# Gorilla-Lab-SCUT/GeoA3

Measured on AMD Instinct MI355X. Metric: attack-iterations/sec (B=250, N=1024), higher is better.
Workload: dtype f32; 1 GPU; configs[1]: PointNet 1024-pt, 250 instances sharded over 1 GPU(s) (250 on rank 0), full GeoA3 (CE + CD 1.0 + HD 0.1 + curvature 1.0 k=16), untargeted; instances_per_gpu=250, global_batch=250, npoint=1024, knn=16, classes=40, wide_mode=f16x2, presteps=150, parallelism=instance-sharded x1

## Files before the change

geoa3_amd/build.py:

```python
from __future__ import annotations

import concurrent.futures
import hashlib
import os
import shutil
import subprocess
import sys

HERE = os.path.dirname(os.path.abspath(__file__))
CSRC = os.path.join(HERE, "csrc")
LIBDIR = os.path.join(HERE, "lib")
OBJDIR = os.path.join(LIBDIR, "obj")
LIB = os.path.join(LIBDIR, "libgeoa3_hip.so")
ARCH = "gfx950"
FLAGS = ["-O3", "-std=c++17", "-fPIC", "--offload-arch=" + ARCH, "-fno-gpu-rdc", "-Wall", "-Wno-unused-function"]


def _hipcc() -> str:
    for c in (os.environ.get("HIPCC"), shutil.which("hipcc"), "/opt/rocm/bin/hipcc"):
        if c and os.path.exists(c):
            return c
    raise RuntimeError("hipcc not found: the HIP library cannot be built")


_NOSLP = ["-fno-slp-vectorize", "-fno-vectorize"]
SLP_FILES = ("pointnet_gemm.hip",)
FILE_FLAGS = {f: list(_NOSLP) for f in sorted(os.listdir(CSRC)) if f.endswith(".hip") and f not in SLP_FILES}
for _f in ("pointnet2_sa.hip", "pointnet2_sa2.hip", "pointnet2_sa2b.hip", "geom_filter.hip", "geom_grid.hip"):
    FILE_FLAGS[_f] = ["-fno-honor-nans"] + _NOSLP


def sources():
    return sorted(os.path.join(CSRC, f) for f in os.listdir(CSRC) if f.endswith(".hip"))


_HIPCC_VERSION = None


def hipcc_version() -> str:
    global _HIPCC_VERSION
    if _HIPCC_VERSION is None:
        r = subprocess.run([_hipcc(), "--version"], capture_output=True, text=True)
        _HIPCC_VERSION = (r.stdout + r.stderr).strip()
    return _HIPCC_VERSION


def _digest(path: str, flags=None) -> str:
    h = hashlib.sha1()
    for p in [path] + sorted(os.path.join(CSRC, f) for f in os.listdir(CSRC) if f.endswith(".h")) + [
            os.path.join(HERE, "..", "include", "geoa3_hip.h"), os.path.join(HERE, "..", "include", "geoa3_hip_debug.h")]:
        with open(p, "rb") as f:
            h.update(f.read())
    h.update(" ".join(flags or FLAGS).encode())
    h.update(hipcc_version().encode())
    h.update(repr((ISA_GUARD_ALL, sorted(ISA_GUARDS.items()))).encode())
    return h.hexdigest()


def _compile(src: str, force: bool, objdir: str = OBJDIR, flags=None) -> str:
    flags_in = tuple(flags or ())
    flags = list(flags or FLAGS)
    if "--no-file-flags" in flags:
        flags.remove("--no-file-flags")
    elif os.path.basename(src) in os.environ.get("GEOA3_NO_FILE_FLAGS_FOR", "").split(",") and objdir != OBJDIR:
        pass
    else:
        flags += FILE_FLAGS.get(os.path.basename(src), [])
    extra = os.environ.get("GEOA3_EXTRA_FILE_FLAGS", "")
    if extra and objdir != OBJDIR:
        names, _, fl = extra.partition(":")
        if os.path.basename(src) in names.split(",") and fl not in flags:
            flags.append(fl)
    obj = os.path.join(objdir, os.path.basename(src) + ".o")
    stamp = obj + ".sha1"
    dig = _digest(src, flags)
    if not force and os.path.exists(obj) and os.path.exists(stamp) and open(stamp).read() == dig:
        return obj
    guarded = ("--no-file-flags" not in (flags_in or ()) and
               not (objdir != OBJDIR and os.environ.get("GEOA3_NO_FILE_FLAGS_FOR")))
    import tempfile
    with tempfile.TemporaryDirectory(dir=objdir) as d:
        tmp_obj = os.path.join(d, os.path.basename(src) + ".o")
        cmd = [_hipcc()] + flags + (["-save-temps=obj"] if guarded else []) + ["-c", src, "-o", tmp_obj]
        r = subprocess.run(cmd, capture_output=True, text=True, cwd=d)
        if r.returncode != 0:
            raise RuntimeError("hipcc failed for %s:\n%s\n%s" % (src, r.stdout, r.stderr))
        if r.stderr.strip():
            sys.stderr.write(r.stderr)
        if guarded:
            base = os.path.splitext(os.path.basename(src))[0]
            asm_file = os.path.join(d, "%s-hip-amdgcn-amd-amdhsa-%s.s" % (base, ARCH))
            if not os.path.exists(asm_file):
                raise RuntimeError("ISA guard: hipcc -save-temps left no device assembly for %s (looked for %s)" % (src, asm_file))
            _isa_guard_asm(src, open(asm_file).read(), flags)
        os.replace(tmp_obj, obj)
    with open(stamp, "w") as f:
        f.write(dig)
    return obj


ISA_GUARDS = {"pointnet_conv_chain.hip": ("conv_bwd_chain_kernel", r"v_pk_(mul|fma|add)_f32"),
              "pointnet2_ops.hip": ("fps_kernel", r"v_pk_(mul|fma|add)_f32"),
              "geom_loss.hip": ("geo_fused_kernel", r"v_pk_(mul|fma|add)_f32")}


ISA_GUARD_ALL = r"(?i)v_pk_(mul|fma|add)_f32\w*[^\n]*\bop_sel\s*[:=]\s*\[[^\]]*1"


GUARD_SELFTEST_SOURCE = r"""
// MUST be refused by the ISA guard: packed FP32 arithmetic whose LOW result reads the HIGH half of a source register pair
#include <hip/hip_runtime.h>
typedef float f2 __attribute__((ext_vector_type(2)));
__global__ void guard_selftest_kernel(const f2* a, const f2* b, f2* out) {
  const int i = blockIdx.x * blockDim.x + threadIdx.x;
  const f2 x = a[i], y = b[i];
  const f2 ys = {y.y, y.x};          // swapped halves: v_pk_fma_f32 ... op_sel:[0,1,0] op_sel_hi:[1,0,1]
  out[i] = x * ys + x;
}
"""


def isa_guard_selftest() -> str:
    import tempfile
    with tempfile.TemporaryDirectory() as d:
        src = os.path.join(d, "guard_selftest.hip")
        with open(src, "w") as f:
            f.write(GUARD_SELFTEST_SOURCE)
        try:
            _isa_guard(src, FLAGS)
        except RuntimeError as e:
            if "ISA guard" in str(e) and "op_sel" in str(e):
                return str(e)
            raise
    raise AssertionError("the ISA guard accepted a source that holds packed FP32 arithmetic with op_sel on a source operand: "
                         "either this hipcc (%s) no longer forms v_pk_*_f32 ... op_sel from the self-test source, or it prints "
                         "it in a way ISA_GUARD_ALL misses -- look at the disassembly before trusting the build"
                         % hipcc_version().splitlines()[0])


def _isa_guard(src: str, flags) -> None:
    import tempfile
    with tempfile.TemporaryDirectory() as d:
        out = os.path.join(d, "guard.s")
        cmd = [_hipcc()] + [f for f in flags if f != "-fPIC"] + ["-S", "--cuda-device-only", "-o", out, src]
        r = subprocess.run(cmd, capture_output=True, text=True)
        if r.returncode != 0:
            raise RuntimeError("ISA guard: hipcc -S failed for %s:\n%s" % (src, r.stderr))
        asm = open(out).read()
    _isa_guard_asm(src, asm, flags)


def _isa_guard_asm(src: str, asm: str, flags) -> None:
    import re
    kernel, pattern = ISA_GUARDS.get(os.path.basename(src), (None, None))
    hit = re.search(ISA_GUARD_ALL, asm)
    if hit:
        raise RuntimeError("ISA guard: %s holds '%s' (NOTEBOOK 5a: packed FP32 with op_sel reads a zero operand in lanes 48-63 "
                           "beside matrix-core wavefronts); keep the two values apart (an opaque asm barrier) or compile the "
                           "file with %s" % (os.path.basename(src), hit.group(0).strip(), " ".join(_NOSLP)))
    if kernel is None:
        return
    found = list(re.finditer(r"^(_Z\w*%s\w*):" % kernel, asm, re.M))
    if not found:
        raise RuntimeError("ISA guard: kernel %s not found in %s" % (kernel, src))
    for m in found:
        body = asm[m.end():]
        body = body[:body.index("s_endpgm")]
        hit = re.search(pattern, body)
        if hit:
            raise RuntimeError("ISA guard: %s holds %s (NOTEBOOK 5a: wrong values beside other wavefronts on its SIMDs); compile "
                               "%s with %s" % (m.group(1), hit.group(0), os.path.basename(src),
                                               FILE_FLAGS.get(os.path.basename(src))))


def build(force: bool = False, verbose: bool = True, extra_flags=(), libdir: str = LIBDIR) -> str:
    objdir, lib = os.path.join(libdir, "obj"), os.path.join(libdir, "libgeoa3_hip.so")
    flags = FLAGS + list(extra_flags)
    os.makedirs(objdir, exist_ok=True)
    srcs = sources()
    with concurrent.futures.ThreadPoolExecutor(max_workers=min(6, len(srcs))) as ex:
        objs = list(ex.map(lambda s: _compile(s, force, objdir, flags), srcs))
    newest = max(os.path.getmtime(o) for o in objs)
    if force or not os.path.exists(lib) or os.path.getmtime(lib) < newest:
        cmd = [_hipcc(), "-shared", "-fPIC", "--offload-arch=" + ARCH, "-o", lib] + objs
        r = subprocess.run(cmd, capture_output=True, text=True)
        if r.returncode != 0:
            raise RuntimeError("link failed:\n%s\n%s" % (r.stdout, r.stderr))
    if verbose:
        print("built", lib, "%.0f KB" % (os.path.getsize(lib) / 1024))
    return lib


if __name__ == "__main__":
    if "--variant" in sys.argv:
        i = sys.argv.index("--variant")
        build(force="--force" in sys.argv, libdir=os.path.abspath(sys.argv[i + 1]),
              extra_flags=[f for f in sys.argv[i + 2:] if f.startswith("-") and f != "--force"])
    else:
        build(force="--force" in sys.argv)
```

geoa3_amd/csrc/pointnet_conv_chain.hip:

```cpp
#include "pointnet_kernels.h"

namespace {

__device__ __forceinline__ void cc_writelane(int& d, int v, int l) {
  asm("v_writelane_b32 %0, %1, %2" : "+v"(d) : "s"(v), "n"(l));
}

constexpr int CC_PITCH = 64 * 2 + 16;
constexpr int CC_BLK = 2 * 64 * CC_PITCH;

__device__ __forceinline__ void cc_mm(const float (&xin)[64], const unsigned char* arow, bool live, f32x16 (&acc)[2][2],
                                      unsigned& Ex) {
#pragma unroll
  for (int c = 0; c < 2; ++c)
#pragma unroll
    for (int t = 0; t < 2; ++t)
#pragma unroll
      for (int r = 0; r < 16; ++r) acc[c][t][r] = 0.f;
  Ex = 14u;
#pragma unroll
  for (int c = 0; c < 4; ++c) {
    const float* x = xin + 16 * c;
    float m = 0.f;
#pragma unroll
    for (int u = 0; u < 16; ++u) m = fmaxf(m, __builtin_fabsf(x[u]));
    const unsigned E = sf_exp(wave_max(live ? m : 0.f));
    if (E > Ex) {
      if (c > 0) {
        const unsigned d = E - Ex;
        const float f = d > 126u ? 0.f : __uint_as_float((127u - d) << 23);
#pragma unroll
        for (int cb = 0; cb < 2; ++cb)
#pragma unroll
          for (int t = 0; t < 2; ++t)
#pragma unroll
            for (int r = 0; r < 16; ++r) acc[cb][t][r] *= f;
      }
      Ex = E;
    }
    const float sx = sf_scale(Ex);
    half8 xh[2], xl[2];
#pragma unroll
    for (int j = 0; j < 8; ++j) {
      float v0 = x[j] * sx, v1 = x[8 + j] * sx;
      geoa3_swap32(v0, v1);
      const _Float16 h0 = (_Float16)v0, h1 = (_Float16)v1;
      xh[0][j] = h0;
      xl[0][j] = (_Float16)(v0 - (float)h0);
      xh[1][j] = h1;
      xl[1][j] = (_Float16)(v1 - (float)h1);
    }
#pragma unroll
    for (int t = 0; t < 2; ++t) {
      const half8 wh = *reinterpret_cast<const half8*>(arow + t * 32 * CC_PITCH + c * 32);
      const half8 wl = *reinterpret_cast<const half8*>(arow + t * 32 * CC_PITCH + c * 32 + 64 * CC_PITCH);
#pragma unroll
      for (int cb = 0; cb < 2; ++cb) {
        acc[cb][t] = __builtin_amdgcn_mfma_f32_32x32x16_f16(wh, xh[cb], acc[cb][t], 0, 0, 0);
        acc[cb][t] = __builtin_amdgcn_mfma_f32_32x32x16_f16(wh, xl[cb], acc[cb][t], 0, 0, 0);
        acc[cb][t] = __builtin_amdgcn_mfma_f32_32x32x16_f16(wl, xh[cb], acc[cb][t], 0, 0, 0);
      }
    }
  }
}

__device__ __forceinline__ void cc_rows(const f32x16 (&acc)[2][2], float (&out)[64]) {
#pragma unroll
  for (int t = 0; t < 2; ++t)
#pragma unroll
    for (int g = 0; g < 4; ++g)
#pragma unroll
      for (int i = 0; i < 4; ++i) {
        float v0 = acc[0][t][4 * g + i], v1 = acc[1][t][4 * g + i];
        geoa3_swap32(v0, v1);
        out[t * 32 + 8 * g + i] = v0;
        out[t * 32 + 8 * g + 4 + i] = v1;
      }
}

__device__ __forceinline__ void cc_wload(const float* W, bool kcontig, int tid, float (&wv)[16], float* s_red) {
  float m = 0.f;
#pragma unroll
  for (int i = 0; i < 16; ++i) {
    wv[i] = W[tid + 256 * i];
    m = fmaxf(m, __builtin_fabsf(wv[i]));
  }
  (void)kcontig;
  m = wave_max(m);
  if ((tid & 63) == 0) s_red[tid >> 6] = m;
}
__device__ __forceinline__ unsigned cc_wsplit(const float (&wv)[16], bool kcontig, int tid, const float* s_red,
                                              unsigned char* s_wh) {
  const unsigned Ew = sf_exp(fmaxf(fmaxf(s_red[0], s_red[1]), fmaxf(s_red[2], s_red[3])));
  const float sw = sf_scale(Ew);
#pragma unroll
  for (int i = 0; i < 16; ++i) {
    const int e = tid + 256 * i;
    const int co = kcontig ? e >> 6 : e & 63, k = kcontig ? e & 63 : e >> 6;
    const float v = wv[i] * sw;
    const _Float16 h = (_Float16)v;
    *reinterpret_cast<_Float16*>(s_wh + co * CC_PITCH + k * 2) = h;
    *reinterpret_cast<_Float16*>(s_wh + 64 * CC_PITCH + co * CC_PITCH + k * 2) = (_Float16)(v - (float)h);
  }
  return Ew;
}

template <int NS, bool FIRST, int COL>
__global__ __launch_bounds__(256) __attribute__((amdgpu_waves_per_eu(2, 2))) void conv_chain_kernel(ConvChainArgs a) {
  extern __shared__ __attribute__((aligned(16))) unsigned char cc_smem[];
  constexpr int NBLK = NS - 1 + COL / 64;
  float4* s_w1 = reinterpret_cast<float4*>(cc_smem + NBLK * CC_BLK);
  float* s_red = reinterpret_cast<float*>(s_w1 + 64);
  const int tid = threadIdx.x, lane = tid & 63, wave = tid >> 6;
  const int b = blockIdx.y;
  const int nblk256 = (a.N + 255) >> 8;
  if (FIRST && tid < 64) s_w1[tid] = make_float4(a.w1[3 * tid], a.w1[3 * tid + 1], a.w1[3 * tid + 2], a.b1[tid]);

  float biasv[NBLK];
  unsigned Ew[NBLK];
  {
    float wv[NBLK][16];
#pragma unroll
    for (int blk = 0; blk < NBLK; ++blk) {
      const int s = blk < NS - 1 ? blk : NS - 1, rb = blk - s;
      const float* W = a.st[s].W + (size_t)b * a.st[s].sWb + (size_t)rb * 4096;
      biasv[blk] = a.st[s].bias[rb * 64 + lane];
      cc_wload(W, true, tid, wv[blk], s_red + blk * 4);
    }
    __syncthreads();
#pragma unroll
    for (int blk = 0; blk < NBLK; ++blk) {
      Ew[blk] = cc_wsplit(wv[blk], true, tid, s_red + blk * 4, cc_smem + blk * CC_BLK);
    }
    __syncthreads();
  }
  for (int cblk = blockIdx.x; cblk < nblk256; cblk += gridDim.x) {
  const int col = cblk * 256 + wave * 64 + lane;
  const bool live = col < a.N, wave_live = cblk * 256 + wave * 64 < a.N;
  const unsigned long long livemask = __builtin_amdgcn_ballot_w64(live);
  const size_t mword = ((size_t)b * ((a.N + 63) >> 6) + (size_t)(cblk * 4 + wave));
  float o[64];
  if (FIRST) {
    const float* xp = a.x3 + (size_t)b * 3 * a.N + (live ? col : a.N - 1);
    const float x0 = xp[0], x1 = xp[a.N], x2 = xp[2 * (size_t)a.N];
    float p0 = x0, p1 = x1, p2 = x2;
    if (a.T3) {
      const float* t = a.T3 + (size_t)b * 9;
      p0 = x0 * t[0] + x1 * t[3] + x2 * t[6];
      p1 = x0 * t[1] + x1 * t[4] + x2 * t[7];
      p2 = x0 * t[2] + x1 * t[5] + x2 * t[8];
    }
#pragma unroll
    for (int u = 0; u < 64; ++u) o[u] = fmaxf(pn_first_layer(s_w1[u], p0, p1, p2), 0.f);
  } else {
    const float* X = a.X + (size_t)b * a.sXb;
    const unsigned xc = (unsigned)(live ? col : a.N - 1);
#pragma unroll
    for (int u = 0; u < 64; ++u) o[u] = (X + (size_t)u * a.ldX)[xc];
  }

#pragma unroll
  for (int blk = 0; blk < NBLK; ++blk) {
    const int s = blk < NS - 1 ? blk : NS - 1, rb = blk - s;
    const bool last = s == NS - 1;
    const ChainStage& st = a.st[s];
    const unsigned char* arow = cc_smem + blk * CC_BLK + (lane & 31) * CC_PITCH + (lane >> 5) * 16;

    f32x16 acc[2][2];
    unsigned Ex;
    cc_mm(o, arow, live, acc, Ex);
    const float unscale = sf_unscale(Ex) * sf_unscale(Ew[blk]);

    float res[64];
    int mlo = 0, mhi = 0;
    cc_rows(acc, res);
#pragma unroll
    for (int row = 0; row < 64; ++row) {
      float r = res[row] * unscale;
      r += __int_as_float(__builtin_amdgcn_readlane(__float_as_int(biasv[blk]), row));
      r = fmaxf(r, 0.f);
      const unsigned long long mk = __builtin_amdgcn_ballot_w64(r > 0.f) & livemask;
      cc_writelane(mlo, (int)(unsigned)mk, row);
      cc_writelane(mhi, (int)(unsigned)(mk >> 32), row);
      res[row] = r;
    }
    if (wave_live)
      st.Ymask[mword * st.Co + rb * 64 + lane] = ((unsigned long long)(unsigned)mhi << 32) | (unsigned)mlo;
    if (st.Y && live) {
      float* Y = st.Y + (size_t)b * st.sYb + (size_t)rb * 64 * a.N;
#pragma unroll
      for (int r = 0; r < 64; ++r) (Y + (size_t)r * a.N)[(unsigned)col] = res[r];
    }
    if (!last) {
#pragma unroll
      for (int r = 0; r < 64; ++r) o[r] = res[r];
    }
  }
  }
}

__global__ __launch_bounds__(256) __attribute__((amdgpu_waves_per_eu(2, 2))) void conv_bwd_chain_kernel(ConvBwdChainArgs a) {
  extern __shared__ __attribute__((aligned(16))) unsigned char cc_smem[];
  float4* s_w1 = reinterpret_cast<float4*>(cc_smem + 3 * CC_BLK);
  float* s_red = reinterpret_cast<float*>(s_w1 + 64);
  float* s_part = s_red + 12;
  const int tid = threadIdx.x, lane = tid & 63, wave = tid >> 6;
  const int cblk = blockIdx.x, b = blockIdx.y;
  const int col = cblk * 256 + wave * 64 + lane;
  const bool live = col < a.N, wave_live = cblk * 256 + wave * 64 < a.N;
  const unsigned xc = (unsigned)(live ? col : a.N - 1);
  const size_t mword = ((size_t)b * ((a.N + 63) >> 6) + (size_t)(cblk * 4 + wave)) * 64;

  float o[64], xb[64];
  {
    const float* X = a.Xa + (size_t)b * 64 * a.N;
#pragma unroll
    for (int u = 0; u < 64; ++u) o[u] = (X + (size_t)u * a.N)[xc];
  }
  const float* xp = a.x3 + (size_t)b * 3 * a.N + xc;
  const float x0 = xp[0], x1 = xp[a.N], x2 = xp[2 * (size_t)a.N];
  float p0 = x0, p1 = x1, p2 = x2;
  if (a.T3) {
    const float* t = a.T3 + (size_t)b * 9;
    p0 = x0 * t[0] + x1 * t[3] + x2 * t[6];
    p1 = x0 * t[1] + x1 * t[4] + x2 * t[7];
    p2 = x0 * t[2] + x1 * t[5] + x2 * t[8];
  }
  if (tid < 64) s_w1[tid] = make_float4(a.w1[3 * tid], a.w1[3 * tid + 1], a.w1[3 * tid + 2], a.b1[tid]);
  const unsigned long long zmv = wave_live ? a.Zmask[mword + lane] : 0ull;

  unsigned Ew[3];
  {
    float wv[3][16];
    cc_wload(a.Wa + (size_t)b * a.sWa, false, tid, wv[0], s_red);
    cc_wload(a.Wb, false, tid, wv[1], s_red + 4);
    cc_wload(a.W2t, true, tid, wv[2], s_red + 8);
    __syncthreads();
    Ew[0] = cc_wsplit(wv[0], false, tid, s_red, cc_smem);
    Ew[1] = cc_wsplit(wv[1], false, tid, s_red + 4, cc_smem + CC_BLK);
    Ew[2] = cc_wsplit(wv[2], true, tid, s_red + 8, cc_smem + 2 * CC_BLK);
    __syncthreads();
  }
  {
    const float* X = a.Xb + (size_t)b * 64 * a.N;
#pragma unroll
    for (int u = 0; u < 64; ++u) xb[u] = (X + (size_t)u * a.N)[xc];
  }
  const unsigned char* arow = cc_smem + (lane & 31) * CC_PITCH + (lane >> 5) * 16;
  f32x16 acc[2][2];
  unsigned Ex;
  float res[64];
  cc_mm(o, arow, live, acc, Ex);
  {
    const float un = sf_unscale(Ex) * sf_unscale(Ew[0]);
    cc_rows(acc, o);
#pragma unroll
    for (int r = 0; r < 64; ++r) o[r] *= un;
  }
  cc_mm(xb, arow + CC_BLK, live, acc, Ex);
  {
    const float un = sf_unscale(Ex) * sf_unscale(Ew[1]);
    cc_rows(acc, res);
    const unsigned sh = lane & 31;
#pragma unroll
    for (int r = 0; r < 64; ++r) {
      float v = res[r] * un;
      v += o[r];
      const unsigned mlo = (unsigned)__builtin_amdgcn_readlane((int)(unsigned)zmv, r);
      const unsigned mhi = (unsigned)__builtin_amdgcn_readlane((int)(unsigned)(zmv >> 32), r);
      o[r] = (((lane < 32 ? mlo : mhi) >> sh) & 1u) ? v : 0.f;
    }
  }
  cc_mm(o, arow + 2 * CC_BLK, live, acc, Ex);
  float q0 = 0.f, q1 = 0.f, q2 = 0.f;
  {
    const float un = sf_unscale(Ex) * sf_unscale(Ew[2]);
    cc_rows(acc, res);
    if (live) {
#pragma unroll
      for (int r = 0; r < 64; ++r) {
        float v = res[r] * un;
        const float4 w = s_w1[r];
        v = pn_first_layer(w, p0, p1, p2) > 0.f ? v : 0.f;
        q0 = fmaf(w.x, v, q0);
        q1 = fmaf(w.y, v, q1);
        q2 = fmaf(w.z, v, q2);
      }
    }
  }
  float d0 = q0, d1 = q1, d2 = q2;
  if (a.T3) {
    const float* t = a.T3 + (size_t)b * 9;
    d0 = fmaf(t[2], q2, fmaf(t[1], q1, t[0] * q0));
    d1 = fmaf(t[5], q2, fmaf(t[4], q1, t[3] * q0));
    d2 = fmaf(t[8], q2, fmaf(t[7], q1, t[6] * q0));
  }
  if (live) {
    float* dxp = a.dx + (size_t)b * 3 * a.N + col;
    dxp[0] = d0;
    dxp[a.N] = d1;
    dxp[2 * (size_t)a.N] = d2;
  }
  if (a.dTpart) {
    const float prod[9] = {x0 * q0, x0 * q1, x0 * q2, x1 * q0, x1 * q1, x1 * q2, x2 * q0, x2 * q1, x2 * q2};
#pragma unroll
    for (int i = 0; i < 9; ++i) {
      const float v = wave_sum(prod[i]);
      if (lane == 0) s_part[wave * 9 + i] = v;
    }
    __syncthreads();
    if (tid < 9) {
      a.dTpart[((size_t)b * gridDim.x + cblk) * GEOA3_DT_PITCH + tid] = s_part[tid] + s_part[9 + tid] + s_part[18 + tid] + s_part[27 + tid];
    }
  }
}

template <int NS, bool FIRST, int COL>
void launch_chain(const ConvChainArgs& a, hipStream_t s) {
  constexpr int NBLK = NS - 1 + COL / 64;
  const size_t lds = (size_t)NBLK * CC_BLK + 64 * 16 + NBLK * 4 * sizeof(float);
  auto kern = conv_chain_kernel<NS, FIRST, COL>;
  (void)hipFuncSetAttribute(reinterpret_cast<const void*>(kern), hipFuncAttributeMaxDynamicSharedMemorySize, (int)lds);
  const int nblk = (a.N + 255) / 256;
  const int gx = (size_t)nblk * a.B > 768 ? (nblk + 1) / 2 : nblk;
  hipLaunchKernelGGL(kern, dim3(gx, a.B), dim3(256), lds, s, a);
}

}

int launch_conv_chain(const ConvChainArgs& a, hipStream_t s) {
  if (a.ns < 1 || a.ns > 3 || a.B <= 0 || a.N <= 0) return GEOA3_EINVAL;
  for (int i = 0; i < a.ns; ++i) {
    if (!a.st[i].W || !a.st[i].bias || !a.st[i].Ymask) return GEOA3_EINVAL;
    if (a.st[i].Co != (i + 1 < a.ns ? 64 : 128)) return GEOA3_ENOSUPPORT;
  }
  const bool first = a.x3 != nullptr;
  if (first ? (!a.w1 || !a.b1) : !a.X) return GEOA3_EINVAL;
  if (a.ns == 3 && first) launch_chain<3, true, 128>(a, s);
  else if (a.ns == 1 && first) launch_chain<1, true, 128>(a, s);
  else if (a.ns == 2 && !first) launch_chain<2, false, 128>(a, s);
  else return GEOA3_ENOSUPPORT;
  GEOA3_CHECK_LAUNCH();
  return GEOA3_OK;
}

int launch_conv_bwd_chain(const ConvBwdChainArgs& a, hipStream_t s) {
  if (!a.Xa || !a.Wa || !a.Xb || !a.Wb || !a.Zmask || !a.W2t || !a.x3 || !a.w1 || !a.b1 || !a.dx || a.B <= 0 || a.N <= 0)
    return GEOA3_EINVAL;
  const size_t lds = (size_t)3 * CC_BLK + 64 * 16 + (12 + 36) * sizeof(float);
  (void)hipFuncSetAttribute(reinterpret_cast<const void*>(conv_bwd_chain_kernel), hipFuncAttributeMaxDynamicSharedMemorySize,
                            (int)lds);
  hipLaunchKernelGGL(conv_bwd_chain_kernel, dim3((a.N + 255) / 256, a.B), dim3(256), lds, s, a);
  GEOA3_CHECK_LAUNCH();
  return GEOA3_OK;
}
```

Baseline: 622.8 iterations/s of a 250-instance batch.

## Use 512-thread workgroups looping over column blocks in PointNet conv chain kernels

For large batches, the forward and backward conv-chain kernels now launch 8-wave workgroups that loop over several column blocks. Each workgroup fetches, scales and splits the per-instance weights into LDS once and reuses them across more columns, which cuts repeated weight loading and setup. The backward kernel now holds the weight preamble once and accumulates dT partials across iterations. The forward epilogue can fuse the Y store into the mask loop when all lanes are live. It also adds compile-time CC_CUT switches for profiling, plus build-guard updates to check both kernel instances. The trade-off is fewer, larger workgroups, which means more register and LDS pressure per group and possibly less occupancy or overlap.

```diff
diff --git a/geoa3_amd/build.py b/geoa3_amd/build.py
--- a/geoa3_amd/build.py
+++ b/geoa3_amd/build.py
@@ -53,7 +53,7 @@
             h.update(f.read())
     h.update(" ".join(flags or FLAGS).encode())
     h.update(hipcc_version().encode())
-    h.update(repr((ISA_GUARD_ALL, sorted(ISA_GUARDS.items()))).encode())
+    h.update(repr((ISA_GUARD_ALL, sorted(ISA_GUARDS.items()), sorted(ISA_GUARD_INSTANCES.items()))).encode())
     return h.hexdigest()
 
 
@@ -69,8 +69,8 @@
     extra = os.environ.get("GEOA3_EXTRA_FILE_FLAGS", "")
     if extra and objdir != OBJDIR:
         names, _, fl = extra.partition(":")
-        if os.path.basename(src) in names.split(",") and fl not in flags:
-            flags.append(fl)
+        if os.path.basename(src) in names.split(","):
+            flags += [f for f in fl.split() if f not in flags]
     obj = os.path.join(objdir, os.path.basename(src) + ".o")
     stamp = obj + ".sha1"
     dig = _digest(src, flags)
@@ -99,9 +99,10 @@
     return obj
 
 
-ISA_GUARDS = {"pointnet_conv_chain.hip": ("conv_bwd_chain_kernel", r"v_pk_(mul|fma|add)_f32"),
+ISA_GUARDS = {"pointnet_conv_chain.hip": (r"conv_bwd_chain(_wg8)?_kernel", r"v_pk_(mul|fma|add)_f32"),
               "pointnet2_ops.hip": ("fps_kernel", r"v_pk_(mul|fma|add)_f32"),
               "geom_loss.hip": ("geo_fused_kernel", r"v_pk_(mul|fma|add)_f32")}
+ISA_GUARD_INSTANCES = {"pointnet_conv_chain.hip": 2}
 
 
 ISA_GUARD_ALL = r"(?i)v_pk_(mul|fma|add)_f32\w*[^\n]*\bop_sel\s*[:=]\s*\[[^\]]*1"
@@ -161,8 +162,9 @@
     if kernel is None:
         return
     found = list(re.finditer(r"^(_Z\w*%s\w*):" % kernel, asm, re.M))
-    if not found:
-        raise RuntimeError("ISA guard: kernel %s not found in %s" % (kernel, src))
+    if len(found) < ISA_GUARD_INSTANCES.get(os.path.basename(src), 1):
+        raise RuntimeError("ISA guard: kernel %s: %d instance(s) found in %s, %d expected" % (
+            kernel, len(found), src, ISA_GUARD_INSTANCES.get(os.path.basename(src), 1)))
     for m in found:
         body = asm[m.end():]
         body = body[:body.index("s_endpgm")]
diff --git a/geoa3_amd/csrc/pointnet_conv_chain.hip b/geoa3_amd/csrc/pointnet_conv_chain.hip
--- a/geoa3_amd/csrc/pointnet_conv_chain.hip
+++ b/geoa3_amd/csrc/pointnet_conv_chain.hip
@@ -1,6 +1,14 @@
 #include "pointnet_kernels.h"
 
+#ifndef GEOA3_CC_CUT
+#define GEOA3_CC_CUT 0
+#endif
+
 namespace {
+
+constexpr int CC_CUT = GEOA3_CC_CUT;
+
+__device__ __forceinline__ void cc_keep(float v) { asm volatile("" ::"v"(v)); }
 
 __device__ __forceinline__ void cc_writelane(int& d, int v, int l) {
   asm("v_writelane_b32 %0, %1, %2" : "+v"(d) : "s"(v), "n"(l));
@@ -78,24 +86,29 @@
       }
 }
 
-__device__ __forceinline__ void cc_wload(const float* W, bool kcontig, int tid, float (&wv)[16], float* s_red) {
+template <int NT>
+__device__ __forceinline__ void cc_wfetch(const float* W, int tid, float (&wv)[4096 / NT]) {
+#pragma unroll
+  for (int i = 0; i < 4096 / NT; ++i) wv[i] = W[tid + NT * i];
+}
+template <int NT>
+__device__ __forceinline__ void cc_wmax(const float (&wv)[4096 / NT], int tid, float* s_red) {
   float m = 0.f;
 #pragma unroll
-  for (int i = 0; i < 16; ++i) {
-    wv[i] = W[tid + 256 * i];
-    m = fmaxf(m, __builtin_fabsf(wv[i]));
-  }
-  (void)kcontig;
+  for (int i = 0; i < 4096 / NT; ++i) m = fmaxf(m, __builtin_fabsf(wv[i]));
   m = wave_max(m);
   if ((tid & 63) == 0) s_red[tid >> 6] = m;
 }
-__device__ __forceinline__ unsigned cc_wsplit(const float (&wv)[16], bool kcontig, int tid, const float* s_red,
+template <int NT>
+__device__ __forceinline__ unsigned cc_wsplit(const float (&wv)[4096 / NT], bool kcontig, int tid, const float* s_red,
                                               unsigned char* s_wh) {
-  const unsigned Ew = sf_exp(fmaxf(fmaxf(s_red[0], s_red[1]), fmaxf(s_red[2], s_red[3])));
+  float wm = fmaxf(fmaxf(s_red[0], s_red[1]), fmaxf(s_red[2], s_red[3]));
+  if (NT == 512) wm = fmaxf(wm, fmaxf(fmaxf(s_red[4], s_red[5]), fmaxf(s_red[6], s_red[7])));
+  const unsigned Ew = sf_exp(wm);
   const float sw = sf_scale(Ew);
 #pragma unroll
-  for (int i = 0; i < 16; ++i) {
-    const int e = tid + 256 * i;
+  for (int i = 0; i < 4096 / NT; ++i) {
+    const int e = tid + NT * i;
     const int co = kcontig ? e >> 6 : e & 63, k = kcontig ? e & 63 : e >> 6;
     const float v = wv[i] * sw;
     const _Float16 h = (_Float16)v;
@@ -105,44 +118,76 @@
   return Ew;
 }
 
-template <int NS, bool FIRST, int COL>
-__global__ __launch_bounds__(256) __attribute__((amdgpu_waves_per_eu(2, 2))) void conv_chain_kernel(ConvChainArgs a) {
+__device__ __forceinline__ void cc_xload(const float* X, size_t ld, unsigned xc, float (&o)[64]) {
+#pragma unroll
+  for (int u = 0; u < 64; ++u) {
+    if (CC_CUT & 2) o[u] = __uint_as_float(0x3c000000u + ((xc & 63u) << 8) + 8192u * (unsigned)u);
+    else o[u] = (X + (size_t)u * ld)[xc];
+  }
+}
+
+template <bool STORE>
+__device__ __forceinline__ void cc_epilogue(float (&res)[64], float unscale, float biasv, unsigned long long livemask, int& mlo,
+                                            int& mhi, float* Y, size_t ldY, unsigned col) {
+#pragma unroll
+  for (int row = 0; row < 64; ++row) {
+    float r = res[row] * unscale;
+    r += __int_as_float(__builtin_amdgcn_readlane(__float_as_int(biasv), row));
+    r = fmaxf(r, 0.f);
+    const unsigned long long mk = __builtin_amdgcn_ballot_w64(r > 0.f) & livemask;
+    cc_writelane(mlo, (int)(unsigned)mk, row);
+    cc_writelane(mhi, (int)(unsigned)(mk >> 32), row);
+    res[row] = r;
+    if (STORE) (Y + (size_t)row * ldY)[col] = r;
+  }
+}
+
+template <int NS, bool FIRST, int COL, int WPG>
+__global__ __launch_bounds__(64 * WPG) __attribute__((amdgpu_waves_per_eu(2, 2))) void conv_chain_kernel(ConvChainArgs a) {
   extern __shared__ __attribute__((aligned(16))) unsigned char cc_smem[];
+  constexpr int NT = 64 * WPG;
   constexpr int NBLK = NS - 1 + COL / 64;
   float4* s_w1 = reinterpret_cast<float4*>(cc_smem + NBLK * CC_BLK);
   float* s_red = reinterpret_cast<float*>(s_w1 + 64);
   const int tid = threadIdx.x, lane = tid & 63, wave = tid >> 6;
   const int b = blockIdx.y;
-  const int nblk256 = (a.N + 255) >> 8;
+  const int nblkw = (a.N + NT - 1) / NT;
+  const bool never = a.N < 0;
   if (FIRST && tid < 64) s_w1[tid] = make_float4(a.w1[3 * tid], a.w1[3 * tid + 1], a.w1[3 * tid + 2], a.b1[tid]);
 
+  float o[64];
   float biasv[NBLK];
   unsigned Ew[NBLK];
-  {
-    float wv[NBLK][16];
+  float wv[NBLK][4096 / NT];
+#pragma unroll
+  for (int blk = 0; blk < NBLK; ++blk) {
+    const int s = blk < NS - 1 ? blk : NS - 1, rb = blk - s;
+    const float* W = a.st[s].W + (size_t)b * a.st[s].sWb + (size_t)rb * 4096;
+    biasv[blk] = a.st[s].bias[rb * 64 + lane];
+    Ew[blk] = 14u;
+    if (!(CC_CUT & 8)) cc_wfetch<NT>(W, tid, wv[blk]);
+  }
+  if (!(CC_CUT & 8)) {
+#pragma unroll
+    for (int blk = 0; blk < NBLK; ++blk) cc_wmax<NT>(wv[blk], tid, s_red + blk * WPG);
+    __syncthreads();
 #pragma unroll
     for (int blk = 0; blk < NBLK; ++blk) {
-      const int s = blk < NS - 1 ? blk : NS - 1, rb = blk - s;
-      const float* W = a.st[s].W + (size_t)b * a.st[s].sWb + (size_t)rb * 4096;
-      biasv[blk] = a.st[s].bias[rb * 64 + lane];
-      cc_wload(W, true, tid, wv[blk], s_red + blk * 4);
+      Ew[blk] = cc_wsplit<NT>(wv[blk], true, tid, s_red + blk * WPG, cc_smem + blk * CC_BLK);
     }
     __syncthreads();
-#pragma unroll
-    for (int blk = 0; blk < NBLK; ++blk) {
-      Ew[blk] = cc_wsplit(wv[blk], true, tid, s_red + blk * 4, cc_smem + blk * CC_BLK);
-    }
-    __syncthreads();
-  }
-  for (int cblk = blockIdx.x; cblk < nblk256; cblk += gridDim.x) {
-  const int col = cblk * 256 + wave * 64 + lane;
-  const bool live = col < a.N, wave_live = cblk * 256 + wave * 64 < a.N;
+  }
+  for (int cblk = blockIdx.x; cblk < nblkw; cblk += gridDim.x) {
+  const int unit = cblk * WPG + wave;
+  const int col = unit * 64 + lane;
+  const bool live = col < a.N, wave_live = unit * 64 < a.N;
+  if (!wave_live) break;
   const unsigned long long livemask = __builtin_amdgcn_ballot_w64(live);
-  const size_t mword = ((size_t)b * ((a.N + 63) >> 6) + (size_t)(cblk * 4 + wave));
-  float o[64];
+  const size_t mword = (size_t)b * ((a.N + 63) >> 6) + (size_t)unit;
   if (FIRST) {
     const float* xp = a.x3 + (size_t)b * 3 * a.N + (live ? col : a.N - 1);
-    const float x0 = xp[0], x1 = xp[a.N], x2 = xp[2 * (size_t)a.N];
+    float x0 = xp[0], x1 = xp[a.N], x2 = xp[2 * (size_t)a.N];
+    if (CC_CUT & 2) x0 = (float)lane, x1 = x0 + 1.f, x2 = x0 + 2.f;
     float p0 = x0, p1 = x1, p2 = x2;
     if (a.T3) {
       const float* t = a.T3 + (size_t)b * 9;
@@ -153,10 +198,7 @@
 #pragma unroll
     for (int u = 0; u < 64; ++u) o[u] = fmaxf(pn_first_layer(s_w1[u], p0, p1, p2), 0.f);
   } else {
-    const float* X = a.X + (size_t)b * a.sXb;
-    const unsigned xc = (unsigned)(live ? col : a.N - 1);
-#pragma unroll
-    for (int u = 0; u < 64; ++u) o[u] = (X + (size_t)u * a.ldX)[xc];
+    cc_xload(a.X + (size_t)b * a.sXb, (size_t)a.ldX, (unsigned)(live ? col : a.N - 1), o);
   }
 
 #pragma unroll
@@ -166,28 +208,28 @@
     const ChainStage& st = a.st[s];
     const unsigned char* arow = cc_smem + blk * CC_BLK + (lane & 31) * CC_PITCH + (lane >> 5) * 16;
 
-    f32x16 acc[2][2];
-    unsigned Ex;
-    cc_mm(o, arow, live, acc, Ex);
-    const float unscale = sf_unscale(Ex) * sf_unscale(Ew[blk]);
-
     float res[64];
     int mlo = 0, mhi = 0;
-    cc_rows(acc, res);
-#pragma unroll
-    for (int row = 0; row < 64; ++row) {
-      float r = res[row] * unscale;
-      r += __int_as_float(__builtin_amdgcn_readlane(__float_as_int(biasv[blk]), row));
-      r = fmaxf(r, 0.f);
-      const unsigned long long mk = __builtin_amdgcn_ballot_w64(r > 0.f) & livemask;
-      cc_writelane(mlo, (int)(unsigned)mk, row);
-      cc_writelane(mhi, (int)(unsigned)(mk >> 32), row);
-      res[row] = r;
-    }
-    if (wave_live)
-      st.Ymask[mword * st.Co + rb * 64 + lane] = ((unsigned long long)(unsigned)mhi << 32) | (unsigned)mlo;
-    if (st.Y && live) {
-      float* Y = st.Y + (size_t)b * st.sYb + (size_t)rb * 64 * a.N;
+    float* Y = st.Y ? st.Y + (size_t)b * st.sYb + (size_t)rb * 64 * a.N : nullptr;
+    bool store = Y && (!(CC_CUT & 1) || never);
+    if (CC_CUT & 4) {
+#pragma unroll
+      for (int r = 0; r < 64; ++r) res[r] = o[r];
+    } else {
+      f32x16 acc[2][2];
+      unsigned Ex;
+      cc_mm(o, arow, live, acc, Ex);
+      const float unscale = sf_unscale(Ex) * sf_unscale(Ew[blk]);
+      cc_rows(acc, res);
+      if (store && livemask == ~0ull) {
+        cc_epilogue<true>(res, unscale, biasv[blk], livemask, mlo, mhi, Y, (size_t)a.N, (unsigned)col);
+        store = false;
+      } else {
+        cc_epilogue<false>(res, unscale, biasv[blk], livemask, mlo, mhi, Y, (size_t)a.N, (unsigned)col);
+      }
+    }
+    st.Ymask[mword * st.Co + rb * 64 + lane] = ((unsigned long long)(unsigned)mhi << 32) | (unsigned)mlo;
+    if (store && live) {
 #pragma unroll
       for (int r = 0; r < 64; ++r) (Y + (size_t)r * a.N)[(unsigned)col] = res[r];
     }
@@ -199,26 +241,56 @@
   }
 }
 
-__global__ __launch_bounds__(256) __attribute__((amdgpu_waves_per_eu(2, 2))) void conv_bwd_chain_kernel(ConvBwdChainArgs a) {
+template <int WPG>
+__device__ __forceinline__ void conv_bwd_chain_body(const ConvBwdChainArgs& a) {
   extern __shared__ __attribute__((aligned(16))) unsigned char cc_smem[];
+  constexpr int NT = 64 * WPG, G = WPG / 4;
   float4* s_w1 = reinterpret_cast<float4*>(cc_smem + 3 * CC_BLK);
   float* s_red = reinterpret_cast<float*>(s_w1 + 64);
-  float* s_part = s_red + 12;
+  float* s_part = s_red + 3 * WPG;
   const int tid = threadIdx.x, lane = tid & 63, wave = tid >> 6;
-  const int cblk = blockIdx.x, b = blockIdx.y;
-  const int col = cblk * 256 + wave * 64 + lane;
-  const bool live = col < a.N, wave_live = cblk * 256 + wave * 64 < a.N;
-  const unsigned xc = (unsigned)(live ? col : a.N - 1);
-  const size_t mword = ((size_t)b * ((a.N + 63) >> 6) + (size_t)(cblk * 4 + wave)) * 64;
-
+  const int b = blockIdx.y;
+  const int nblkw = (a.N + NT - 1) / NT, nparts = (a.N + 255) >> 8;
+  const bool never = a.N < 0;
+  const float* XA = a.Xa + (size_t)b * 64 * a.N;
+  const float* XB = a.Xb + (size_t)b * 64 * a.N;
+
+  unsigned Ew[3] = {14u, 14u, 14u};
+  float wv[3][4096 / NT];
+  if (!(CC_CUT & 8)) {
+    cc_wfetch<NT>(a.Wa + (size_t)b * a.sWa, tid, wv[0]);
+    cc_wfetch<NT>(a.Wb, tid, wv[1]);
+    cc_wfetch<NT>(a.W2t, tid, wv[2]);
+  }
+  if (tid < 64) s_w1[tid] = make_float4(a.w1[3 * tid], a.w1[3 * tid + 1], a.w1[3 * tid + 2], a.b1[tid]);
   float o[64], xb[64];
   {
-    const float* X = a.Xa + (size_t)b * 64 * a.N;
-#pragma unroll
-    for (int u = 0; u < 64; ++u) o[u] = (X + (size_t)u * a.N)[xc];
-  }
+    const int col = blockIdx.x * NT + wave * 64 + lane;
+    const unsigned xc = (unsigned)(col < a.N ? col : a.N - 1);
+    cc_xload(XA, (size_t)a.N, xc, o);
+  }
+  if (!(CC_CUT & 8)) {
+    cc_wmax<NT>(wv[0], tid, s_red);
+    cc_wmax<NT>(wv[1], tid, s_red + WPG);
+    cc_wmax<NT>(wv[2], tid, s_red + 2 * WPG);
+    __syncthreads();
+    Ew[0] = cc_wsplit<NT>(wv[0], false, tid, s_red, cc_smem);
+    Ew[1] = cc_wsplit<NT>(wv[1], false, tid, s_red + WPG, cc_smem + CC_BLK);
+    Ew[2] = cc_wsplit<NT>(wv[2], true, tid, s_red + 2 * WPG, cc_smem + 2 * CC_BLK);
+  }
+  __syncthreads();
+
+  int it = 0;
+  for (int cblk = blockIdx.x; cblk < nblkw; cblk += gridDim.x, ++it) {
+  const int unit = cblk * WPG + wave;
+  const int col = unit * 64 + lane;
+  const bool live = col < a.N, wave_live = unit * 64 < a.N;
+  const unsigned xc = (unsigned)(live ? col : a.N - 1);
+  const size_t mword = ((size_t)b * ((a.N + 63) >> 6) + (size_t)unit) * 64;
+  if (it > 0) cc_xload(XA, (size_t)a.N, xc, o);
   const float* xp = a.x3 + (size_t)b * 3 * a.N + xc;
-  const float x0 = xp[0], x1 = xp[a.N], x2 = xp[2 * (size_t)a.N];
+  float x0 = xp[0], x1 = xp[a.N], x2 = xp[2 * (size_t)a.N];
+  if (CC_CUT & 2) x0 = (float)lane, x1 = x0 + 1.f, x2 = x0 + 2.f;
   float p0 = x0, p1 = x1, p2 = x2;
   if (a.T3) {
     const float* t = a.T3 + (size_t)b * 9;
@@ -226,27 +298,20 @@
     p1 = x0 * t[1] + x1 * t[4] + x2 * t[7];
     p2 = x0 * t[2] + x1 * t[5] + x2 * t[8];
   }
-  if (tid < 64) s_w1[tid] = make_float4(a.w1[3 * tid], a.w1[3 * tid + 1], a.w1[3 * tid + 2], a.b1[tid]);
-  const unsigned long long zmv = wave_live ? a.Zmask[mword + lane] : 0ull;
-
-  unsigned Ew[3];
-  {
-    float wv[3][16];
-    cc_wload(a.Wa + (size_t)b * a.sWa, false, tid, wv[0], s_red);
-    cc_wload(a.Wb, false, tid, wv[1], s_red + 4);
-    cc_wload(a.W2t, true, tid, wv[2], s_red + 8);
-    __syncthreads();
-    Ew[0] = cc_wsplit(wv[0], false, tid, s_red, cc_smem);
-    Ew[1] = cc_wsplit(wv[1], false, tid, s_red + 4, cc_smem + CC_BLK);
-    Ew[2] = cc_wsplit(wv[2], true, tid, s_red + 8, cc_smem + 2 * CC_BLK);
-    __syncthreads();
-  }
-  {
-    const float* X = a.Xb + (size_t)b * 64 * a.N;
-#pragma unroll
-    for (int u = 0; u < 64; ++u) xb[u] = (X + (size_t)u * a.N)[xc];
-  }
+  unsigned long long zmv = wave_live ? a.Zmask[mword + lane] : 0ull;
+  if (CC_CUT & 2) zmv = 0x5555555555555555ull * (unsigned)(lane + 1);
+  cc_xload(XB, (size_t)a.N, xc, xb);
+
   const unsigned char* arow = cc_smem + (lane & 31) * CC_PITCH + (lane >> 5) * 16;
+  float q0 = 0.f, q1 = 0.f, q2 = 0.f;
+  if (CC_CUT & 4) {
+#pragma unroll
+    for (int r = 0; r < 64; ++r) {
+      cc_keep(o[r]);
+      cc_keep(xb[r]);
+    }
+    q0 = o[0], q1 = xb[0], q2 = p0 + p1 + p2 + (float)(unsigned)zmv;
+  } else {
   f32x16 acc[2][2];
   unsigned Ex;
   float res[64];
@@ -272,7 +337,6 @@
     }
   }
   cc_mm(o, arow + 2 * CC_BLK, live, acc, Ex);
-  float q0 = 0.f, q1 = 0.f, q2 = 0.f;
   {
     const float un = sf_unscale(Ex) * sf_unscale(Ew[2]);
     cc_rows(acc, res);
@@ -288,6 +352,7 @@
       }
     }
   }
+  }
   float d0 = q0, d1 = q1, d2 = q2;
   if (a.T3) {
     const float* t = a.T3 + (size_t)b * 9;
@@ -295,7 +360,7 @@
     d1 = fmaf(t[5], q2, fmaf(t[4], q1, t[3] * q0));
     d2 = fmaf(t[8], q2, fmaf(t[7], q1, t[6] * q0));
   }
-  if (live) {
+  if (live && (!(CC_CUT & 1) || never)) {
     float* dxp = a.dx + (size_t)b * 3 * a.N + col;
     dxp[0] = d0;
     dxp[a.N] = d1;
@@ -306,24 +371,47 @@
 #pragma unroll
     for (int i = 0; i < 9; ++i) {
       const float v = wave_sum(prod[i]);
-      if (lane == 0) s_part[wave * 9 + i] = v;
-    }
+      if (lane == 0) s_part[((it & 1) * WPG + wave) * 9 + i] = v;
+    }
+  }
+  }
+  if (a.dTpart) {
     __syncthreads();
-    if (tid < 9) {
-      a.dTpart[((size_t)b * gridDim.x + cblk) * GEOA3_DT_PITCH + tid] = s_part[tid] + s_part[9 + tid] + s_part[18 + tid] + s_part[27 + tid];
-    }
-  }
+    if (tid < 2 * G * 9) {
+      const int i = tid % 9, g = (tid / 9) % G, t = tid / (9 * G);
+      const int cblk = blockIdx.x + t * gridDim.x, part = cblk * G + g;
+      if (cblk < nblkw && part < nparts) {
+        const float* sp = s_part + (t * WPG + 4 * g) * 9 + i;
+        a.dTpart[((size_t)b * nparts + part) * GEOA3_DT_PITCH + i] = sp[0] + sp[9] + sp[18] + sp[27];
+      }
+    }
+  }
+}
+
+__global__ __launch_bounds__(256) __attribute__((amdgpu_waves_per_eu(2, 2))) void conv_bwd_chain_kernel(ConvBwdChainArgs a) {
+  conv_bwd_chain_body<4>(a);
+}
+__global__ __launch_bounds__(512) __attribute__((amdgpu_waves_per_eu(2, 2))) void conv_bwd_chain_wg8_kernel(ConvBwdChainArgs a) {
+  conv_bwd_chain_body<8>(a);
+}
+
+constexpr size_t CC_BIG_BLOCKS = 768;
+
+template <int NS, bool FIRST, int COL, int WPG>
+void launch_chain_form(const ConvChainArgs& a, int gx, hipStream_t s) {
+  constexpr int NBLK = NS - 1 + COL / 64;
+  const size_t lds = (size_t)NBLK * CC_BLK + 64 * 16 + NBLK * WPG * sizeof(float);
+  auto kern = conv_chain_kernel<NS, FIRST, COL, WPG>;
+  (void)hipFuncSetAttribute(reinterpret_cast<const void*>(kern), hipFuncAttributeMaxDynamicSharedMemorySize, (int)lds);
+  hipLaunchKernelGGL(kern, dim3(gx, a.B), dim3(64 * WPG), lds, s, a);
 }
 
 template <int NS, bool FIRST, int COL>
 void launch_chain(const ConvChainArgs& a, hipStream_t s) {
-  constexpr int NBLK = NS - 1 + COL / 64;
-  const size_t lds = (size_t)NBLK * CC_BLK + 64 * 16 + NBLK * 4 * sizeof(float);
-  auto kern = conv_chain_kernel<NS, FIRST, COL>;
-  (void)hipFuncSetAttribute(reinterpret_cast<const void*>(kern), hipFuncAttributeMaxDynamicSharedMemorySize, (int)lds);
   const int nblk = (a.N + 255) / 256;
-  const int gx = (size_t)nblk * a.B > 768 ? (nblk + 1) / 2 : nblk;
-  hipLaunchKernelGGL(kern, dim3(gx, a.B), dim3(256), lds, s, a);
+  const bool big = (size_t)nblk * a.B > CC_BIG_BLOCKS;
+  if (big) launch_chain_form<NS, FIRST, COL, 8>(a, ((a.N + 511) / 512 + 1) / 2, s);
+  else launch_chain_form<NS, FIRST, COL, 4>(a, nblk, s);
 }
 
 }
@@ -347,10 +435,13 @@
 int launch_conv_bwd_chain(const ConvBwdChainArgs& a, hipStream_t s) {
   if (!a.Xa || !a.Wa || !a.Xb || !a.Wb || !a.Zmask || !a.W2t || !a.x3 || !a.w1 || !a.b1 || !a.dx || a.B <= 0 || a.N <= 0)
     return GEOA3_EINVAL;
-  const size_t lds = (size_t)3 * CC_BLK + 64 * 16 + (12 + 36) * sizeof(float);
-  (void)hipFuncSetAttribute(reinterpret_cast<const void*>(conv_bwd_chain_kernel), hipFuncAttributeMaxDynamicSharedMemorySize,
-                            (int)lds);
-  hipLaunchKernelGGL(conv_bwd_chain_kernel, dim3((a.N + 255) / 256, a.B), dim3(256), lds, s, a);
+  const int nblk = (a.N + 255) / 256;
+  const bool big = (size_t)nblk * a.B > CC_BIG_BLOCKS;
+  const int wpg = big ? 8 : 4;
+  const size_t lds = (size_t)3 * CC_BLK + 64 * 16 + (3 * wpg + 2 * wpg * 9) * sizeof(float);
+  auto kern = big ? conv_bwd_chain_wg8_kernel : conv_bwd_chain_kernel;
+  (void)hipFuncSetAttribute(reinterpret_cast<const void*>(kern), hipFuncAttributeMaxDynamicSharedMemorySize, (int)lds);
+  hipLaunchKernelGGL(kern, dim3(big ? ((a.N + 511) / 512 + 1) / 2 : nblk, a.B), dim3(64 * wpg), lds, s, a);
   GEOA3_CHECK_LAUNCH();
   return GEOA3_OK;
 }
```

Result: no change. 628.2 iterations/s of a 250-instance batch (median of 6 runs) (+0.9%).
